# jpe17/TwoTowerMLRetrieval

Hardware: AMD Instinct MI355X
Metric: queries/sec top-k over 10M x 256-d docs (higher is better)
Workload: dtype f32 results (bit-identical to the fp32 FMA chain); f16-MFMA screen + fp32 rescoring

## Files before the change

### twotowermlretrieval_amd/csrc/score_topk.hip

```cpp
#include "tt_common.h"

#include <limits.h>
#include <math.h>

namespace {

constexpr int TILE_DOCS = 32;
constexpr int SLAB_BYTES = 32 * 128;
constexpr int NSTAGE = 4;
#ifndef TT_K4_NT_NSTAGE
#define TT_K4_NT_NSTAGE 4
#endif
constexpr int NSTAGE_NT = TT_K4_NT_NSTAGE;
constexpr int WPB = 4;
constexpr int DMA_PER_SLAB = 4;
constexpr int PACE_R = 16;
constexpr int PACE_POLLS = 400;
constexpr int DRAW_POLLS = 1 << 16;
constexpr int DRAW_GAVE_UP = 0x7fffffff;

typedef __attribute__((address_space(3))) void lds_void;
typedef const __attribute__((address_space(1))) void gbl_void;

struct Cand;
// ... 701 lines not shown
        for (int u = 0; u < MERGE_SEG / MERGE_THREADS; ++u) {
            const int m = base + tid + u * MERGE_THREADS;
            ci[u] = m < end ? ix_at(m) : -1;
        }
#pragma unroll
        for (int u = 0; u < MERGE_SEG / MERGE_THREADS; ++u) {
            if (ci[u] >= 0) {
                const int slot = atomicAdd(&pool_n, 1);
                pool_v[slot] = v_at(base + tid + u * MERGE_THREADS);
                pool_i[slot] = ci[u];
            }
        }
        __syncthreads();
    }
    const int kept = reduce_pool();
    if (tid < k) {
        out_val[(size_t)b * k + tid] = tid < kept ? pool_v[tid] : -INFINITY;
        out_idx[(size_t)b * k + tid] = tid < kept ? pool_i[tid] : -1;
    }
}

__device__ __forceinline__ unsigned order_key(float f)
{
    const unsigned b = __float_as_uint(f);
    return (b & 0x80000000u) ? ~b : (b | 0x80000000u);
}

__device__ __forceinline__ float order_key_to_float(unsigned key)
{
    return __uint_as_float((key & 0x80000000u) ? (key & 0x7fffffffu) : ~key);
}

__global__ __launch_bounds__(256) void kth_largest_kernel(const float *__restrict__ vals, int M, int k,
                                                          float *__restrict__ out, const int *run_if,
                                                          float *__restrict__ top_out)
{
    if (run_if && run_if[blockIdx.x >> 5] == 0)
        return;
    __shared__ int hist[256];
    __shared__ int sel[2];
    __shared__ int wpos;
    const int row = blockIdx.x, tid = threadIdx.x, lane = tid & 63;
    const float *v = vals + (size_t)row * M;
    if (M < k) {
        if (tid == 0 && out)
            out[row] = -INFINITY;
        if (top_out)
            for (int i = tid; i < k; i += 256)
                top_out[(size_t)row * k + i] = i < M ? v[i] : -INFINITY;
        return;
    }
    unsigned prefix = 0u, mask = 0u;
    int k_rem = k;
    constexpr int KTH_REG = 16;
    const bool in_regs = M <= 256 * KTH_REG;
    unsigned keys[KTH_REG];
    if (in_regs) {
#pragma unroll
        for (int i = 0; i < KTH_REG; ++i) {
            const int m = tid + 256 * i;
            keys[i] = m < M ? order_key(v[m]) : 0u;
        }
    }
#pragma unroll 1
    for (int pass = 0; pass < 4; ++pass) {
        const int shift = 24 - 8 * pass;
        hist[tid] = 0;
        __syncthreads();
        if (in_regs) {
#pragma unroll
            for (int i = 0; i < KTH_REG; ++i)
                if (tid + 256 * i < M && (keys[i] & mask) == prefix)
                    atomicAdd(&hist[(keys[i] >> shift) & 255u], 1);
        } else {
            for (int m = tid; m < M; m += 256) {
                const unsigned key = order_key(v[m]);
                if ((key & mask) == prefix)
                    atomicAdd(&hist[(key >> shift) & 255u], 1);
            }
        }
        __syncthreads();
        if (tid < 64) {
            int c[4], s = 0;
#pragma unroll
            for (int i = 0; i < 4; ++i) {
                c[i] = hist[255 - (lane * 4 + i)];
                s += c[i];
            }
            int incl = s;
#pragma unroll
            for (int off = 1; off < 64; off <<= 1) {
                const int y = __shfl_up(incl, off);
                if (lane >= off)
                    incl += y;
            }
            int above = incl - s;
#pragma unroll
            for (int i = 0; i < 4; ++i) {
                if (above < k_rem && above + c[i] >= k_rem) {
                    sel[0] = 255 - (lane * 4 + i);
                    sel[1] = above;
                }
                above += c[i];
            }
        }
        __syncthreads();
        prefix |= (unsigned)sel[0] << shift;
        mask |= 0xffu << shift;
        k_rem -= sel[1];
        __syncthreads();
    }
    const float kth = order_key_to_float(prefix);
    if (tid == 0 && out)
        out[row] = kth;
    if (top_out) {
        if (tid == 0)
            wpos = 0;
        __syncthreads();
        float *dst = top_out + (size_t)row * k;
        if (in_regs) {
#pragma unroll
            for (int i = 0; i < KTH_REG; ++i)
                if (tid + 256 * i < M && keys[i] > prefix)
                    dst[atomicAdd(&wpos, 1)] = order_key_to_float(keys[i]);
        } else {
            for (int m = tid; m < M; m += 256)
// ... 636 lines not shown
```

### twotowermlretrieval_amd/csrc/screen.hip

```cpp
#include "tt_common.h"
#include <cmath>

#include <hip/hip_fp16.h>
#include <limits.h>
#include <math.h>

int tt_score_topk_f32_pred(const float *Q, int B, int d, const float *D, int64_t N, int k, int64_t idx_offset,
                           float *out_val, int64_t *out_idx, void *workspace, size_t workspace_bytes,
                           const int *run_if, hipStream_t st);

int tt_kth_largest(const float *vals, int B, int M, int k, float *out, hipStream_t st);
int tt_k_largest_list(const float *vals, int B, int M, int k, float *list, hipStream_t st);

namespace {

typedef _Float16 h8 __attribute__((ext_vector_type(8)));
typedef _Float16 h4 __attribute__((ext_vector_type(4)));
typedef __attribute__((address_space(3))) void lds_void;
typedef const __attribute__((address_space(1))) void gbl_void;

#ifndef TT_SCREEN_STAGGER
#define TT_SCREEN_STAGGER 1
#endif
constexpr int SW = 8;
constexpr int STILE_BYTES = 32 * 512;
constexpr int SRING = 8;
constexpr int STPB = 2;
constexpr int SCAP = 128;
constexpr int SURV_MAX = 1024;
constexpr int POOL_MAX = 8192;
constexpr int FIN_MAX_CHUNKS = 2048;

struct SCand {
    float v;
    int x;
};

__device__ __forceinline__ float screen_eps(float qnorm, float dmax)
{
    return 1.10e-3f * qnorm * dmax + 1e-6f * (qnorm + dmax);
}

__device__ __forceinline__ SCand scand_load_l2(const SCand *p)
{
    unsigned long long u = __hip_atomic_load((const unsigned long long *)p, __ATOMIC_RELAXED, __HIP_MEMORY_SCOPE_AGENT);
    SCand c;
    c.v = __uint_as_float((unsigned)u);
    c.x = (int)(u >> 32);
    return c;
}

struct ScreenParams {
    const float *Q;
    const _Float16 *D16;
    int B, N, k;
    int n_chunks, tiles_per_chunk, n_tiles;
    int static_tiles, tail_g, tail_blocks;
    int *tail_ctr;
    float dmax;
    SCand *cand;
    int *pcnt;
    int *flag;
    float *max_val;
    const float *thr0;
    int thr0_stride;
    const h8 *qimg;
    const float *qnorm;
    const float *dbg_thr;
};

__device__ __forceinline__ void scand_store_async(const SCand *base, unsigned byte_off, float v, int x)
{
    const unsigned long long bits = ((unsigned long long)(unsigned)x << 32) | (unsigned long long)__float_as_uint(v);
    asm volatile("global_store_dwordx2 %0, %1, %2\n\ts_nop 1" ::"v"(byte_off), "v"(bits), "s"(base) : "memory");
}

__device__ __forceinline__ void f32_store_async(float *dst, float v)
{
    asm volatile("global_store_dword %0, %1, off\n\ts_nop 0" ::"v"(dst), "v"(v) : "memory");
}

constexpr int SQUART = SCAP / 4;
constexpr int SQ_TRIGGER = SQUART - 10;
constexpr int SQ_KEEP_MAX = 4 * SQ_TRIGGER - 4;

__device__ __forceinline__ void screen_compact(SCand *base, const int (&n)[4], int k, float slack, int lane, int &n_new,
                                               float &thr_new, bool &have, bool &overflow)
{
    float v[2];
    int x[2], rank[2];
    bool live[2];
#pragma unroll
    for (int i = 0; i < 2; ++i) {
        v[i] = -INFINITY;
        x[i] = INT_MAX;
        rank[i] = 0;
        live[i] = (lane & 31) < ((lane >> 5) ? n[2 * i + 1] : n[2 * i]);
        if (live[i]) {
            const SCand c = scand_load_l2(base + 64 * i + lane);
            v[i] = c.v;
            x[i] = c.x;
        }
    }
#pragma unroll
    for (int i2 = 0; i2 < 2; ++i2) {
#pragma unroll
        for (int sub = 0; sub < 2; ++sub) {
            const int lim = n[2 * i2 + sub];
            for (int l2 = 0; l2 < lim; ++l2) {
                const float sv = __builtin_bit_cast(float, __builtin_amdgcn_readlane(__builtin_bit_cast(int, v[i2]), 32 * sub + l2));
                const int sx = __builtin_amdgcn_readlane(x[i2], 32 * sub + l2);
#pragma unroll
                for (int i = 0; i < 2; ++i)
                    rank[i] += (sv > v[i] || (sv == v[i] && sx < x[i])) ? 1 : 0;
            }
        }
// ... 118 lines not shown
                            : INFINITY;
        float c_init = -t_init;
        if (MAXONLY)
            c_init = (p.dbg_thr && live) ? -p.dbg_thr[qrow] : 0.0f;
        negthr[c] = f32x4{c_init, c_init, c_init, c_init};
    }

    SCand *const cwave = p.cand + ((size_t)blockIdx.x * QB + w * QW) * SCAP;

    auto compact_where = [&](int c, unsigned qmask) {
        asm volatile("s_waitcnt vmcnt(0)" ::: "memory");
        while (qmask) {
            const int q = __ffs((int)qmask) - 1;
            qmask &= qmask - 1;
            const int nq[4] = {__builtin_amdgcn_readlane(cnt[c], q), __builtin_amdgcn_readlane(cnt[c], q + 16),
                               __builtin_amdgcn_readlane(cnt[c], q + 32), __builtin_amdgcn_readlane(cnt[c], q + 48)};
            const float slack = __builtin_bit_cast(float, __builtin_amdgcn_readlane(__builtin_bit_cast(int, eps2[c]), q));
            int n_new;
            float tn;
            bool have, ovf;
            screen_compact(cwave + (size_t)(16 * c + q) * SCAP, nq, k, slack, lane, n_new, tn, have, ovf);
            if (ovf && lane == 0)
                atomicOr(p.flag + ((qbase + 16 * c) >> 5), 1);
            if (n == q) {
                cnt[c] = (n_new - g + 3) >> 2;
                if (have)
                    negthr[c] = f32x4{-tn, -tn, -tn, -tn};
            }
        }
    };

    const char *D = (const char *)p.D16;
    const char *rowp[2];
    auto set_rows = [&](int tile) {
#pragma unroll
        for (int i = 0; i < 2; ++i) {
            const int row = 2 * (2 * w + i) + (lane >> 5);
            const int doc = min(tile * 32 + row, p.N - 1);
            const int chunk16 = (lane & 31) ^ (row & 15);
            rowp[i] = D + (size_t)doc * 512 + chunk16 * 16;
        }
    };
    auto dma_issue = [&](int tile, int stage) {
        set_rows(min(tile, t1 - 1));
        char *dst = ring + stage * STILE_BYTES + (2 * w) * 1024;
        __builtin_amdgcn_global_load_lds((gbl_void *)rowp[0], (lds_void *)dst, 16, 0, DMA_AUX);
        __builtin_amdgcn_global_load_lds((gbl_void *)rowp[1], (lds_void *)(dst + 1024), 16, 0, DMA_AUX);
    };
    auto dma_piece = [&](int i, int stage) {
        char *dst = ring + stage * STILE_BYTES + (2 * w + i) * 1024;
        __builtin_amdgcn_global_load_lds((gbl_void *)rowp[i], (lds_void *)dst, 16, 0, DMA_AUX);
    };

    for (;;) {
    if (t0 < t1) {
#pragma unroll
        for (int gi = 0; gi < SRING - STPB; ++gi)
            dma_issue(t0 + gi, gi);
        int stage = 0;
        const int rd_base = n * 512;
        f32x4 acc[2][NSET];
        const bool late = TT_SCREEN_STAGGER && w >= 4;
        bool pending = false;
        int ptile = 0;
        auto epilogue = [&](int tile) {
                const int tile_base = tile * 32;
            const bool partial = tile_base + 32 > p.N;
            if (!MAXONLY) {
                if (partial) {
#pragma unroll
                    for (int u = 0; u < 2; ++u)
#pragma unroll
                        for (int r = 0; r < 4; ++r)
                            if (tile_base + 16 * u + 4 * g + r >= p.N) {
#pragma unroll
                                for (int c = 0; c < NSET; ++c)
                                    acc[u][c][r] = -INFINITY;
                            }
                }
                int mall = INT_MIN;
#pragma unroll
                for (int u = 0; u < 2; ++u)
#pragma unroll
                    for (int c = 0; c < NSET; ++c)
#pragma unroll
                        for (int r = 0; r < 4; ++r)
                            mall = max(mall, __float_as_int(acc[u][c][r]));
                if (__ballot(mall >= 0) != 0ull) {
#pragma unroll
                    for (int c = 0; c < NSET; ++c) {
                        int mu[2];
#pragma unroll
                        for (int u = 0; u < 2; ++u)
                            mu[u] = max(max(__float_as_int(acc[u][c][0]), __float_as_int(acc[u][c][1])),
                                        max(__float_as_int(acc[u][c][2]), __float_as_int(acc[u][c][3])));
                        if (__ballot(max(mu[0], mu[1]) >= 0) == 0ull)
                            continue;
                        const unsigned mine = (unsigned)(((16 * c + n) * SCAP + SQUART * g) * sizeof(SCand));
                        const float thr_c = -negthr[c][0];
#pragma unroll
                        for (int u = 0; u < 2; ++u) {
                            if (__ballot(mu[u] >= 0) == 0ull)
                                continue;
#pragma unroll
                            for (int r = 0; r < 4; ++r) {
                                if (__float_as_int(acc[u][c][r]) >= 0) {
                                    scand_store_async(cwave, mine + (unsigned)cnt[c] * (unsigned)sizeof(SCand),
                                                      acc[u][c][r] + thr_c, tile_base + 16 * u + 4 * g + r);
                                    ++cnt[c];
                                }
                            }
                        }
                        unsigned long long full = __ballot(cnt[c] > SQ_TRIGGER);
                        full = (full | (full >> 32));
                        full = (full | (full >> 16)) & 0xffffull;
                        if (full)
                            compact_where(c, (unsigned)full);
                    }
                }
            } else {
#pragma unroll
                for (int c = 0; c < NSET; ++c) {
                    float m = -INFINITY;
                    if (!partial) {
                        int mi = INT_MIN;
#pragma unroll
                        for (int u = 0; u < 2; ++u)
#pragma unroll
                            for (int r = 0; r < 4; ++r)
                                mi = max(mi, __float_as_int(acc[u][c][r]));
                        m = __int_as_float(mi);
                    } else {
#pragma unroll
                        for (int u = 0; u < 2; ++u)
#pragma unroll
                            for (int r = 0; r < 4; ++r)
                                m = fmaxf(m, tile_base + 16 * u + 4 * g + r < p.N ? acc[u][c][r] : -INFINITY);
                    }
                    m = fmaxf(m, __shfl_xor(m, 16));
                    m = fmaxf(m, __shfl_xor(m, 32));
                    const int qrow = qbase + 16 * c + n;
                    if (g == 0 && qrow < p.B)
                        f32_store_async(p.max_val + (size_t)qrow * p.n_tiles + tile, m);
                }
            }
                };
        for (int tile = t0; tile < t1; ++tile) {
            if ((tile - t0) % STPB == 0) {
                asm volatile("s_waitcnt vmcnt(%0)" ::"n"(2 * (SRING - 2 * STPB)) : "memory");
                __builtin_amdgcn_s_barrier();
            }
            const int fill_stage = (stage + SRING - STPB) % SRING;
            set_rows(min(tile + SRING - STPB, t1 - 1));
            if (!wave_live) {
                dma_piece(0, fill_stage);
                dma_piece(1, fill_stage);
            }
            if (wave_live) {
                if (late && pending)
                    epilogue(ptile);
                const char *buf = ring + stage * STILE_BYTES + rd_base;
                h8 a0[3], a1[3];
                auto a_read = [&](int s) {
                    const int off = ((4 * s + g) ^ n) << 4;
                    a0[s % 3] = *(const h8 *)(buf + off);
                    a1[s % 3] = *(const h8 *)(buf + 16 * 512 + off);
                };
                a_read(0);
                a_read(1);
#pragma unroll
                for (int s = 0; s < 8; ++s) {
                    if (s + 2 < 8)
                        a_read(s + 2);
                    if (s == 2)
                        dma_piece(0, fill_stage);
                    if (s == 6)
                        dma_piece(1, fill_stage);
                    __builtin_amdgcn_sched_barrier(0);
#pragma unroll
                    for (int c = 0; c < NSET; ++c) {
                        const f32x4 c0 = s == 0 ? negthr[c] : acc[0][c];
                        const f32x4 c1 = s == 0 ? negthr[c] : acc[1][c];
                        acc[0][c] = __builtin_amdgcn_mfma_f32_16x16x32_f16(a0[s % 3], qreg[c][s], c0, 0, 0, 0);
                        acc[1][c] = __builtin_amdgcn_mfma_f32_16x16x32_f16(a1[s % 3], qreg[c][s], c1, 0, 0, 0);
                    }
                    __builtin_amdgcn_sched_barrier(0);
                }
                if (late) {
                    pending = true;
                    ptile = tile;
                } else {
                    epilogue(tile);
                }
            }
            stage = (stage + 1) % SRING;
        }
// ... 222 lines not shown
                    const int qrow = qbase + 16 * c + n;
                    if (g == 0 && qrow < p.B)
                        f32_store_async(p.max_val + (size_t)qrow * p.n_tiles + tile, m);
                }
            }
        }
    }
    asm volatile("s_waitcnt vmcnt(0)" ::: "memory");
    if (MAXONLY)
        return;
#pragma unroll
    for (int c = 0; c < NQS; ++c) {
        int tot = cnt[c] + __shfl_xor(cnt[c], 16);
        tot += __shfl_xor(tot, 32);
        const unsigned long long over = __ballot(tot > k) & 0xffffull;
        if (over)
            compact_where(c, (unsigned)over);
        int packed = cnt[c] << (8 * g);
        packed |= __shfl_xor(packed, 16);
        packed |= __shfl_xor(packed, 32);
        const int qrow = qbase + 16 * c + n;
        if (g == 0 && qrow < p.B)
            p.pcnt[(size_t)qrow * p.n_chunks + chunk] = packed;
    }
}

struct FinishParams {
    const float *Q;
    const float *D32;
    int B, N, k, n_chunks;
    float dmax;
    const SCand *cand;
    const int *pcnt;
    int *flag;
    int64_t idx_offset;
    float *out_val;
    int64_t *out_idx;
    int q_per_block;
    int *stats;
};

__device__ __forceinline__ bool before_f(float sa, int ia, float sb, int ib) { return sa > sb || (sa == sb && ia < ib); }

__device__ __forceinline__ unsigned f32_order_key(float f)
{
    const unsigned b = __float_as_uint(f);
    return (b & 0x80000000u) ? ~b : (b | 0x80000000u);
}
__device__ __forceinline__ float f32_from_order_key(unsigned k)
{
    return __uint_as_float((k & 0x80000000u) ? (k & 0x7fffffffu) : ~k);
}

__global__ __launch_bounds__(256) void screen_finish_kernel(FinishParams p)
{
    __shared__ float pool_v[POOL_MAX];
    __shared__ float qs[256];
    __shared__ float sv_v[SURV_MAX];
    __shared__ int sv_x[SURV_MAX];
    __shared__ float red_v[4];
    __shared__ int hist[256];
    extern __shared__ int fin_dyn[];
    int *const ccnt = fin_dyn;
    int *const pre = fin_dyn + p.n_chunks;
    __shared__ int sel[2];
    __shared__ int n_pool, n_surv;
    const int row = blockIdx.x, tid = threadIdx.x;
    if (tid == 0)
        n_pool = n_surv = 0;
    qs[tid] = p.Q[(size_t)row * 256 + tid];
    __syncthreads();
    float ss = qs[tid] * qs[tid];
#pragma unroll
    for (int off = 32; off >= 1; off >>= 1)
        ss += __shfl_xor(ss, off);
    if ((tid & 63) == 0)
        red_v[tid >> 6] = ss;
    __syncthreads();
    const float eps2 = 2.0f * screen_eps(sqrtf(red_v[0] + red_v[1] + red_v[2] + red_v[3]), p.dmax);
    __syncthreads();

    const int qgroup = row / p.q_per_block, qin = row % p.q_per_block;
    bool too_many = false;
    const int per = (p.n_chunks + 255) / 256;
    {
        int sum = 0;
        for (int c = tid * per; c < min(tid * per + per, p.n_chunks); ++c) {
            const int v = p.pcnt[(size_t)row * p.n_chunks + c];
            ccnt[c] = v;
            sum += (v & 0xff) + ((v >> 8) & 0xff) + ((v >> 16) & 0xff) + ((v >> 24) & 0xff);
        }
        int inc = sum;
#pragma unroll
        for (int off = 1; off < 64; off <<= 1) {
            const int v = __shfl_up(inc, off);
            if ((tid & 63) >= off)
                inc += v;
        }
        if ((tid & 63) == 63)
            hist[tid >> 6] = inc;
        __syncthreads();
        int base = 0;
        for (int wv = 0; wv < (tid >> 6); ++wv)
            base += hist[wv];
        if (tid == 255)
            n_pool = base + inc;
        __syncthreads();
        hist[tid] = base + inc - sum;
    }
    __syncthreads();
    {
        int run = hist[tid];
        for (int c = tid * per; c < min(tid * per + per, p.n_chunks); ++c) {
            pre[c] = run;
            const int v = ccnt[c];
            run += (v & 0xff) + ((v >> 8) & 0xff) + ((v >> 16) & 0xff) + ((v >> 24) & 0xff);
        }
        if (tid == 255)
            pre[p.n_chunks] = n_pool;
    }
    __syncthreads();
    const int total = n_pool;
    if (total > POOL_MAX)
        too_many = true;
    auto locate = [&](int m) -> const SCand * {
        int lo = 0, hi = p.n_chunks;
        while (hi - lo > 1) {
            const int mid = (lo + hi) >> 1;
            if (pre[mid] <= m)
                lo = mid;
            else
                hi = mid;
        }
        int o = m - pre[lo], slot = 0;
#pragma unroll
        for (int gq = 0; gq < 4; ++gq) {
            const int ng = (ccnt[lo] >> (8 * gq)) & 0xff;
            if (o >= 0 && o < ng)
                slot = SQUART * gq + o;
            o -= ng;
            if (o < 0)
                o = INT_MIN / 2;
        }
        return p.cand + ((size_t)(qgroup * p.n_chunks + lo) * p.q_per_block + qin) * SCAP + slot;
// ... 13 lines not shown
            hist[tid] = 0;
            __syncthreads();
            for (int m = tid; m < np; m += 256) {
                const unsigned key = f32_order_key(pool_v[m]);
                if ((key & mask) == prefix)
                    atomicAdd(&hist[(key >> shift) & 255u], 1);
            }
            __syncthreads();
            if (tid < 64) {
                const int ln = tid;
                int c[4], sm = 0;
#pragma unroll
                for (int i = 0; i < 4; ++i) {
                    c[i] = hist[255 - (ln * 4 + i)];
                    sm += c[i];
                }
                int incl = sm;
#pragma unroll
                for (int off = 1; off < 64; off <<= 1) {
                    const int y = __shfl_up(incl, off);
                    if (ln >= off)
                        incl += y;
                }
                int above = incl - sm;
#pragma unroll
                for (int i = 0; i < 4; ++i) {
                    if (above < k_rem && above + c[i] >= k_rem) {
                        sel[0] = 255 - (ln * 4 + i);
                        sel[1] = above;
                    }
                    above += c[i];
                }
            }
            __syncthreads();
            prefix |= (unsigned)sel[0] << shift;
            mask |= 0xffu << shift;
            k_rem -= sel[1];
            __syncthreads();
        }
        kth = f32_from_order_key(prefix);
    }
    const float cut = found == p.k ? kth - eps2 : -INFINITY;
    for (int m = tid; m < np; m += 256) {
        if (pool_v[m] >= cut) {
            const int slot = atomicAdd(&n_surv, 1);
            if (slot < SURV_MAX)
                sv_x[slot] = locate(m)->x;
            else
                too_many = true;
        }
    }
    __syncthreads();
    const int ns = min(n_surv, SURV_MAX);
    for (int sidx = tid; sidx < ns; sidx += 256) {
        const float *drow = p.D32 + (size_t)sv_x[sidx] * 256;
        float acc = 0.0f;
#pragma unroll 1
        for (int x0 = 0; x0 < 256; x0 += 64) {
            f32x4 dv[16];
#pragma unroll
            for (int i = 0; i < 16; ++i)
                dv[i] = __builtin_nontemporal_load((const f32x4 *)(drow + x0 + 4 * i));
#pragma unroll
            for (int i = 0; i < 16; ++i) {
                acc = fmaf(qs[x0 + 4 * i], dv[i].x, acc);
                acc = fmaf(qs[x0 + 4 * i + 1], dv[i].y, acc);
                acc = fmaf(qs[x0 + 4 * i + 2], dv[i].z, acc);
                acc = fmaf(qs[x0 + 4 * i + 3], dv[i].w, acc);
            }
        }
        sv_v[sidx] = acc;
    }
    if (tid == 0) {
        p.stats[2 * row] = n_pool;
        p.stats[2 * row + 1] = n_surv;
    }
    if (__syncthreads_or(too_many) && tid == 0)
        atomicOr(p.flag + (row >> 5), 4);
    __syncthreads();
    for (int sidx = tid; sidx < ns; sidx += 256) {
        const float mv = sv_v[sidx];
        const int mx = sv_x[sidx];
        int rank = 0;
        for (int u = 0; u < ns; ++u)
            rank += before_f(sv_v[u], sv_x[u], mv, mx) ? 1 : 0;
        if (rank < p.k) {
            p.out_val[(size_t)row * p.k + rank] = mv;
            p.out_idx[(size_t)row * p.k + rank] = p.idx_offset + mx;
        }
    }
    for (int r = ns + tid; r < p.k; r += 256) {
        p.out_val[(size_t)row * p.k + r] = -INFINITY;
        p.out_idx[(size_t)row * p.k + r] = -1;
    }
}

__global__ __launch_bounds__(256) void build_f16_kernel(const float *__restrict__ D, int64_t N, int d,
                                                        _Float16 *__restrict__ out, unsigned *__restrict__ stats)
{
    __shared__ float red[8];
    const int lane = threadIdx.x & 63, wave = threadIdx.x >> 6;
    float nmax = 0.0f, amax = 0.0f;
    for (int64_t row = (int64_t)blockIdx.x * 4 + wave; row < N; row += (int64_t)gridDim.x * 4) {
        float ss = 0.0f;
        for (int x = lane * 4; x < d; x += 256) {
            const f32x4 v = *(const f32x4 *)(D + row * d + x);
            h4 hv;
#pragma unroll
            for (int e = 0; e < 4; ++e) {
                ss += v[e] * v[e];
                amax = fmaxf(amax, fabsf(v[e]));
                if (!(fabsf(v[e]) <= 3.0e38f))
                    amax = INFINITY;
                hv[e] = (_Float16)v[e];
            }
            *(h4 *)(out + row * d + x) = hv;
        }
#pragma unroll
        for (int off = 32; off >= 1; off >>= 1)
            ss += __shfl_xor(ss, off);
        nmax = fmaxf(nmax, sqrtf(ss));
    }
#pragma unroll
    for (int off = 32; off >= 1; off >>= 1)
// ... 17 lines not shown
    const int lane = threadIdx.x & 63, wave = threadIdx.x >> 6;
    float nmax = 0.0f, amax = 0.0f;
    for (int64_t row = (int64_t)blockIdx.x * 4 + wave; row < N; row += (int64_t)gridDim.x * 4) {
        float ss = 0.0f;
        for (int x = lane * 4; x < d; x += 256) {
            const uint2 raw = *(const uint2 *)(S + row * d + x);
            f32x4 v;
            v[0] = __uint_as_float(raw.x << 16);
            v[1] = __uint_as_float(raw.x & 0xffff0000u);
            v[2] = __uint_as_float(raw.y << 16);
            v[3] = __uint_as_float(raw.y & 0xffff0000u);
            h4 hv;
#pragma unroll
            for (int e = 0; e < 4; ++e) {
                ss += v[e] * v[e];
                amax = fmaxf(amax, fabsf(v[e]));
                if (!(fabsf(v[e]) <= 3.0e38f))
                    amax = INFINITY;
                hv[e] = (_Float16)v[e];
            }
            *(f32x4 *)(out32 + row * d + x) = v;
            if (out16)
                *(h4 *)(out16 + row * d + x) = hv;
        }
#pragma unroll
        for (int off = 32; off >= 1; off >>= 1)
            ss += __shfl_xor(ss, off);
        nmax = fmaxf(nmax, sqrtf(ss));
    }
#pragma unroll
    for (int off = 32; off >= 1; off >>= 1)
        amax = fmaxf(amax, __shfl_xor(amax, off));
    if (lane == 0) {
        red[wave] = nmax;
        red[4 + wave] = amax;
    }
    __syncthreads();
    if (threadIdx.x == 0 && stats) {
        atomicMax(stats, __float_as_uint(fmaxf(fmaxf(red[0], red[1]), fmaxf(red[2], red[3]))));
        atomicMax(stats + 1, __float_as_uint(fmaxf(fmaxf(red[4], red[5]), fmaxf(red[6], red[7]))));
    }
}

struct SPlan {
    bool stream;
    int nset;
    int n_qgroups;
    int q_per_block;
    int n_tiles, n_chunks, tiles_per_chunk, n_blocks;
    int static_tiles, tail_g, tail_blocks;
    size_t tailctr_off;
    bool sample;
    int s_tiles, s_chunks, s_tiles_per_chunk, s_blocks;
    int64_t s_docs;
    size_t cand_off, pcnt_off, smax_val_off, sthr_val_off, qimg_off, qnorm_off, stats_off, ws_bytes, lds;
    int rows_pad;
};

constexpr int64_t SAMPLE_MIN_N = 65536;
constexpr int STREAM_MAX_B = 64;

int screen_cus()
{
    int dev = 0, cus = 0;
    if (hipGetDevice(&dev) != hipSuccess ||
        hipDeviceGetAttribute(&cus, hipDeviceAttributeMultiprocessorCount, dev) != hipSuccess || cus <= 0) {
        (void)hipGetLastError();
        cus = 256;
    }
    return cus;
}

SPlan make_splan(int B, int64_t N, int k)
{
    SPlan pl;
    pl.stream = B <= STREAM_MAX_B;
    if (B <= SW * 32) {
        pl.nset = B <= SW * 16 ? 1 : 2;
    } else {
        const int groups = (B + SW * 64 - 1) / (SW * 64);
        pl.nset = (B + groups - 1) / groups <= SW * 48 ? 3 : 4;
    }
    pl.q_per_block = pl.stream ? (B <= 32 ? 32 : 64) : SW * 16 * pl.nset;
    pl.n_qgroups = (B + pl.q_per_block - 1) / pl.q_per_block;
    pl.n_tiles = (int)((N + 31) / 32);
    int want, max_chunks;
    if (pl.stream) {
        want = (screen_cus() * 2 * TW + pl.n_qgroups - 1) / pl.n_qgroups;
        max_chunks = N >= SAMPLE_MIN_N ? FIN_MAX_CHUNKS : POOL_MAX / (k + 16);
    } else {
        want = (screen_cus() + pl.n_qgroups - 1) / pl.n_qgroups;
        max_chunks = POOL_MAX / (k + 16);
        max_chunks = max_chunks > 255 ? 255 : max_chunks;
    }
    want = want > max_chunks ? max_chunks : want;
    want = want > pl.n_tiles ? pl.n_tiles : want;
    want = want < 1 ? 1 : want;
    pl.tiles_per_chunk = (pl.n_tiles + want - 1) / want;
    pl.n_chunks = (pl.n_tiles + pl.tiles_per_chunk - 1) / pl.tiles_per_chunk;
    pl.static_tiles = pl.n_tiles;
    pl.tail_g = 1;
    pl.tail_blocks = 0;
    {
        const int tail_div = TT_AB_SWITCH(TT_SCREEN_TAIL_DIV, 8);
        const int share = tail_div > 0 ? pl.tiles_per_chunk / tail_div : 0;
        if (!pl.stream && share >= 16) {
            const int own = pl.tiles_per_chunk - share;
            int g = share / 4;
            g = g < 8 ? 8 : (g > 32 ? 32 : g);
            pl.tiles_per_chunk = own;
            pl.static_tiles = own * pl.n_chunks < pl.n_tiles ? own * pl.n_chunks : pl.n_tiles;
            pl.tail_g = g;
            pl.tail_blocks = (pl.n_tiles - pl.static_tiles + g - 1) / g;
        }
    }
    const int n_tasks = pl.n_qgroups * pl.n_chunks;
    pl.n_blocks = pl.stream ? (n_tasks + TW - 1) / TW : n_tasks;
    const size_t rows = (size_t)pl.n_qgroups * pl.q_per_block;
    size_t off = 0;
    pl.cand_off = off;
    off = tt_align_up(off + (size_t)n_tasks * pl.q_per_block * SCAP * sizeof(SCand), 256);
    pl.pcnt_off = off;
    off = tt_align_up(off + rows * pl.n_chunks * sizeof(int), 256);
    pl.sample = N >= SAMPLE_MIN_N;
    int64_t s_docs = N / 64;
    const int per_k = k <= 16 ? 4096 : 2048;
    const int64_t s_min = (int64_t)k * per_k < N / 4 ? (int64_t)k * per_k : N / 4;
    s_docs = s_docs < s_min ? s_min : s_docs;
    s_docs = s_docs < 32 ? 32 : s_docs;
    pl.s_docs = (s_docs + 31) / 32 * 32;
    pl.s_tiles = (int)(pl.s_docs / 32);
    int s_want = pl.stream ? (screen_cus() * 2 * TW + pl.n_qgroups - 1) / pl.n_qgroups
                           : (screen_cus() + pl.n_qgroups - 1) / pl.n_qgroups;
    s_want = s_want > pl.s_tiles ? pl.s_tiles : s_want;
    s_want = s_want < 1 ? 1 : s_want;
    pl.s_tiles_per_chunk = (pl.s_tiles + s_want - 1) / s_want;
    pl.s_chunks = pl.sample ? (pl.s_tiles + pl.s_tiles_per_chunk - 1) / pl.s_tiles_per_chunk : 0;
    pl.s_blocks = pl.stream ? (pl.n_qgroups * pl.s_chunks + TW - 1) / TW : pl.n_qgroups * pl.s_chunks;
    pl.smax_val_off = off;
    off = tt_align_up(off + rows * (size_t)(pl.sample ? pl.s_tiles : 1) * sizeof(float), 256);
    pl.sthr_val_off = off;
    off = tt_align_up(off + rows * sizeof(float), 256);
    pl.rows_pad = (int)rows;
    pl.qimg_off = off;
    off = tt_align_up(off + rows * 256 * sizeof(_Float16), 256);
    pl.qnorm_off = off;
    off = tt_align_up(off + rows * sizeof(float), 256);
    pl.tailctr_off = off;
    off = tt_align_up(off + (size_t)pl.n_qgroups * sizeof(int), 256);
    pl.stats_off = off;
    off = tt_align_up(off + rows * 2 * sizeof(int), 256);
    pl.ws_bytes = off;
    pl.lds = pl.stream ? (size_t)TW * TSTAGE * TSLAB_BYTES : (size_t)SRING * STILE_BYTES;
    return pl;
}

}

TT_EXPORT int tt_index_build_f16(const float *D, int64_t N, int d, void *D16, float *stats, tt_stream_t stream)
{
    if (N < 0 || d <= 0 || (d & 3))
        return tt_fail(TT_ERR_BAD_SHAPE, "tt_index_build_f16: N=%lld d=%d", (long long)N, d);
    if (!stats || (N > 0 && (!D || !D16)))
        return tt_fail(TT_ERR_BAD_SHAPE, "tt_index_build_f16: null pointer");
    hipStream_t st = (hipStream_t)stream;
    TT_RC_CHECK(tt_zero_async(stats, 2 * sizeof(float), st));
    if (N == 0)
        return TT_OK;
    const int64_t want_blocks = (N + 3) / 4;
    hipLaunchKernelGGL(build_f16_kernel, dim3((unsigned)(want_blocks > 8192 ? 8192 : want_blocks)), dim3(256), 0, st, D,
                       N, d, (_Float16 *)D16, (unsigned *)stats);
    TT_LAUNCH_CHECK();
    return TT_OK;
}

TT_EXPORT int tt_index_build_from_bf16(const void *D_bf16, int64_t N, int d, float *D32, void *D16, float *stats,
                                       int reset_stats, tt_stream_t stream)
{
    if (N < 0 || d <= 0 || (d & 3))
        return tt_fail(TT_ERR_BAD_SHAPE, "tt_index_build_from_bf16: N=%lld d=%d", (long long)N, d);
    if (N > 0 && (!D_bf16 || !D32))
        return tt_fail(TT_ERR_BAD_SHAPE, "tt_index_build_from_bf16: null pointer");
    hipStream_t st = (hipStream_t)stream;
    if (stats && reset_stats)
        TT_RC_CHECK(tt_zero_async(stats, 2 * sizeof(float), st));
    if (N == 0)
        return TT_OK;
    const int64_t want_blocks = (N + 3) / 4;
    hipLaunchKernelGGL(build_from_bf16_kernel, dim3((unsigned)(want_blocks > 8192 ? 8192 : want_blocks)), dim3(256), 0,
                       st, (const unsigned short *)D_bf16, N, d, D32, (_Float16 *)D16, (unsigned *)stats);
    TT_LAUNCH_CHECK();
    return TT_OK;
}
// ... 14 lines not shown
}

namespace {
__global__ void seed_fill_kernel(float *seed, int n)
{
    const int i = blockIdx.x * 256 + threadIdx.x;
    if (i < n)
        seed[i] = -3.0e38f;
}

int screened_impl(const char *who, int phase, const float *Q, int B, int d, const float *D32, const void *D16, int64_t N, int k,
                  int k_seed, float dmax_norm, int64_t idx_offset, float *out_val, int64_t *out_idx, int32_t *fallback_flag,
                  float *seed, void *workspace, size_t workspace_bytes, void *const *prof_events, hipStream_t st)
{
    if (B <= 0 || N <= 0 || k <= 0)
        return tt_fail(TT_ERR_BAD_SHAPE, "%s: B=%d N=%lld k=%d", who, B, (long long)N, k);
    if (d != 256)
        return tt_fail(TT_ERR_UNSUPPORTED, "%s: d=%d (supported: 256)", who, d);
    if (k > 64)
        return tt_fail(TT_ERR_UNSUPPORTED, "%s: k=%d > 64", who, k);
    if (N >= (int64_t)INT_MAX - 64)
        return tt_fail(TT_ERR_UNSUPPORTED, "%s: N too large; shard the corpus", who);
    if (!(dmax_norm >= 0.0f) || !(dmax_norm < 60000.0f))
        return tt_fail(TT_ERR_UNSUPPORTED, "%s: corpus norm %g outside the fp16 range", who, dmax_norm);
    const bool seed_only = phase == 1 || phase == 3;
    if (!Q || !D16 || !fallback_flag || (!seed_only && (!D32 || !out_val || !out_idx)) || (phase != 0 && !seed))
        return tt_fail(TT_ERR_BAD_SHAPE, "%s: null pointer", who);
    if (seed_only && (k_seed < 1 || k_seed > k))
        return tt_fail(TT_ERR_BAD_SHAPE, "%s: k_seed=%d outside [1, k=%d]", who, k_seed, k);
    const SPlan pl = make_splan(B, N, k);
    const size_t need = pl.ws_bytes + tt_score_topk_workspace_bytes(B, N, d, k);
    if (!workspace || workspace_bytes < need || ((uintptr_t)workspace & 255))
        return tt_fail(TT_ERR_WORKSPACE, "%s: workspace %zu < %zu bytes", who, workspace_bytes, need);
    char *ws = (char *)workspace;

    ScreenParams sp;
    sp.Q = Q;
    sp.D16 = (const _Float16 *)D16;
    sp.B = B;
    sp.N = (int)N;
    sp.k = k;
    sp.n_chunks = pl.n_chunks;
    sp.tiles_per_chunk = pl.tiles_per_chunk;
    sp.n_tiles = pl.n_tiles;
    sp.static_tiles = pl.static_tiles;
    sp.tail_g = pl.tail_g;
    sp.tail_blocks = pl.tail_blocks;
    sp.tail_ctr = (int *)(ws + pl.tailctr_off);
    sp.dmax = dmax_norm;
    sp.cand = (SCand *)(ws + pl.cand_off);
    sp.pcnt = (int *)(ws + pl.pcnt_off);
    sp.flag = fallback_flag;
    sp.max_val = nullptr;
    sp.thr0 = nullptr;
    sp.thr0_stride = k;
    sp.qimg = (const h8 *)(ws + pl.qimg_off);
    sp.qnorm = (const float *)(ws + pl.qnorm_off);
    sp.dbg_thr = nullptr;
    if (phase != 2) {
        hipLaunchKernelGGL(q_image_kernel, dim3(pl.rows_pad / 32), dim3(128), 0, st, Q, B, (h8 *)(ws + pl.qimg_off),
                           (float *)(ws + pl.qnorm_off), fallback_flag, (B + 31) / 32, (int *)(ws + pl.tailctr_off),
                           pl.n_qgroups);
        TT_LAUNCH_CHECK();
    }
    auto launch = [&](const ScreenParams &a, int blocks, bool maxonly) -> int {
        if (pl.stream && pl.q_per_block == 64) {
            if (maxonly)
                hipLaunchKernelGGL((screen_stream_kernel<true, 4>), dim3(blocks), dim3(TW * 64), pl.lds, st, a);
            else
                hipLaunchKernelGGL((screen_stream_kernel<false, 4>), dim3(blocks), dim3(TW * 64), pl.lds, st, a);
        } else if (pl.stream) {
            if (maxonly)
                hipLaunchKernelGGL(screen_stream_kernel<true>, dim3(blocks), dim3(TW * 64), pl.lds, st, a);
            else
                hipLaunchKernelGGL(screen_stream_kernel<false>, dim3(blocks), dim3(TW * 64), pl.lds, st, a);
        } else if (pl.nset == 4) {
            if (maxonly)
                hipLaunchKernelGGL((screen_kernel<true, 4>), dim3(blocks), dim3(SW * 64), pl.lds, st, a);
            else
                hipLaunchKernelGGL((screen_kernel<false, 4>), dim3(blocks), dim3(SW * 64), pl.lds, st, a);
        } else if (pl.nset == 3) {
            if (maxonly)
                hipLaunchKernelGGL((screen_kernel<true, 3>), dim3(blocks), dim3(SW * 64), pl.lds, st, a);
            else
                hipLaunchKernelGGL((screen_kernel<false, 3>), dim3(blocks), dim3(SW * 64), pl.lds, st, a);
        } else if (pl.nset == 2) {
            if (maxonly)
                hipLaunchKernelGGL((screen_kernel<true, 2>), dim3(blocks), dim3(SW * 64), pl.lds, st, a);
            else
                hipLaunchKernelGGL((screen_kernel<false, 2>), dim3(blocks), dim3(SW * 64), pl.lds, st, a);
        } else {
            if (maxonly)
                hipLaunchKernelGGL((screen_kernel<true, 1>), dim3(blocks), dim3(SW * 64), pl.lds, st, a);
            else
                hipLaunchKernelGGL((screen_kernel<false, 1>), dim3(blocks), dim3(SW * 64), pl.lds, st, a);
        }
        TT_LAUNCH_CHECK();
        return TT_OK;
    };
    if (pl.stream && pl.q_per_block == 64) {
        TT_HIP_CHECK(hipFuncSetAttribute((const void *)screen_stream_kernel<false, 4>, hipFuncAttributeMaxDynamicSharedMemorySize, (int)pl.lds));
        TT_HIP_CHECK(hipFuncSetAttribute((const void *)screen_stream_kernel<true, 4>, hipFuncAttributeMaxDynamicSharedMemorySize, (int)pl.lds));
    } else if (pl.stream) {
        TT_HIP_CHECK(hipFuncSetAttribute((const void *)screen_stream_kernel<false>, hipFuncAttributeMaxDynamicSharedMemorySize, (int)pl.lds));
        TT_HIP_CHECK(hipFuncSetAttribute((const void *)screen_stream_kernel<true>, hipFuncAttributeMaxDynamicSharedMemorySize, (int)pl.lds));
    } else {
        const void *fns[8] = {(const void *)screen_kernel<false, 4>, (const void *)screen_kernel<true, 4>,
                              (const void *)screen_kernel<false, 2>, (const void *)screen_kernel<true, 2>,
                              (const void *)screen_kernel<false, 1>, (const void *)screen_kernel<true, 1>,
                              (const void *)screen_kernel<false, 3>, (const void *)screen_kernel<true, 3>};
        const int f0 = pl.nset == 4 ? 0 : (pl.nset == 2 ? 2 : (pl.nset == 3 ? 6 : 4));
        TT_HIP_CHECK(hipFuncSetAttribute(fns[f0], hipFuncAttributeMaxDynamicSharedMemorySize, (int)pl.lds));
        TT_HIP_CHECK(hipFuncSetAttribute(fns[f0 + 1], hipFuncAttributeMaxDynamicSharedMemorySize, (int)pl.lds));
    }
    if (phase == 2) {
        sp.thr0 = seed;
        sp.thr0_stride = 1;
    } else if (!pl.sample && seed_only) {
        const int n = phase == 3 ? B * k_seed : B;
        hipLaunchKernelGGL(seed_fill_kernel, dim3((n + 255) / 256), dim3(256), 0, st, seed, n);
        TT_LAUNCH_CHECK();
    } else if (pl.sample) {
        ScreenParams ss = sp;
        ss.N = (int)pl.s_docs;
        ss.n_tiles = pl.s_tiles;
        ss.n_chunks = pl.s_chunks;
        ss.tiles_per_chunk = pl.s_tiles_per_chunk;
        ss.static_tiles = pl.s_tiles;
        ss.tail_blocks = 0;
        ss.max_val = (float *)(ws + pl.smax_val_off);
        int rc = launch(ss, pl.s_blocks, true);
        if (rc != TT_OK)
            return rc;
        if (phase == 3)
            rc = tt_k_largest_list(ss.max_val, B, pl.s_tiles, k_seed, seed, st);
        else
            rc = tt_kth_largest(ss.max_val, B, pl.s_tiles, phase == 1 ? k_seed : k, phase == 1 ? seed : (float *)(ws + pl.sthr_val_off), st);
        if (rc != TT_OK)
            return rc;
        sp.thr0 = (const float *)(ws + pl.sthr_val_off);
        sp.thr0_stride = 1;
    }
    if (seed_only)
        return TT_OK;
    if (prof_events)
        TT_HIP_CHECK(hipEventRecord((hipEvent_t)prof_events[0], st));
    {
        const int rc = launch(sp, pl.n_blocks, false);
        if (rc != TT_OK)
            return rc;
    }
    if (prof_events)
        TT_HIP_CHECK(hipEventRecord((hipEvent_t)prof_events[1], st));

    FinishParams fp;
    fp.Q = Q;
    fp.D32 = D32;
    fp.B = B;
    fp.N = (int)N;
    fp.k = k;
    fp.n_chunks = pl.n_chunks;
    fp.q_per_block = pl.q_per_block;
    fp.dmax = dmax_norm;
    fp.cand = sp.cand;
    fp.pcnt = sp.pcnt;
    fp.flag = fallback_flag;
    fp.idx_offset = idx_offset;
    fp.out_val = out_val;
    fp.out_idx = out_idx;
    fp.stats = (int *)(ws + pl.stats_off);
    hipLaunchKernelGGL(screen_finish_kernel, dim3(B), dim3(256), (size_t)(2 * pl.n_chunks + 1) * sizeof(int), st, fp);
    TT_LAUNCH_CHECK();
    return tt_score_topk_f32_pred(Q, B, d, D32, N, k, idx_offset, out_val, out_idx, ws + pl.ws_bytes,
                                  workspace_bytes - pl.ws_bytes, fallback_flag, st);
}
}

TT_EXPORT int tt_score_topk_screened_f32(const float *Q, int B, int d, const float *D32, const void *D16, int64_t N,
                                         int k, float dmax_norm, int64_t idx_offset, float *out_val, int64_t *out_idx,
                                         int32_t *fallback_flag, void *workspace, size_t workspace_bytes,
                                         void *const *prof_events, tt_stream_t stream)
{
    return screened_impl("tt_score_topk_screened_f32", 0, Q, B, d, D32, D16, N, k, k, dmax_norm, idx_offset, out_val, out_idx,
                         fallback_flag, nullptr, workspace, workspace_bytes, prof_events, (hipStream_t)stream);
}

TT_EXPORT int tt_score_topk_screened_seed_f32(const float *Q, int B, int d, const void *D16, int64_t N, int k, int k_seed,
                                              float dmax_norm, int32_t *fallback_flag, float *seed, void *workspace,
                                              size_t workspace_bytes, tt_stream_t stream)
{
// ... 40 lines not shown
    pl.n_chunks = (pl.n_tiles + pl.tiles_per_chunk - 1) / pl.tiles_per_chunk;
    const int n_tasks = pl.n_qgroups * pl.n_chunks;
    pl.n_blocks = form == 0 ? (n_tasks + TW - 1) / TW : n_tasks;
    size_t off = 0;
    pl.qimg_off = off;
    off = tt_align_up(off + (size_t)pl.rows_pad * 256 * sizeof(_Float16), 256);
    pl.qnorm_off = off;
    off = tt_align_up(off + (size_t)pl.rows_pad * sizeof(float), 256);
    pl.flag_off = off;
    off = tt_align_up(off + (size_t)(pl.rows_pad / 32 + 1) * sizeof(int), 256);
    pl.total = off;
    return true;
}
}

TT_EXPORT size_t tt_debug_screen_s16_workspace_bytes(int B, int64_t N, int form)
{
    DbgPlan pl;
    if (B <= 0 || N <= 0 || !make_dbg_plan(B, N, form, pl))
        return 0;
    return pl.total;
}

TT_EXPORT int tt_debug_screen_s16(const float *Q, int B, const void *D16, int64_t N, float dmax_norm, const float *thr,
                                  int form, float *out_t, void *workspace, size_t workspace_bytes, tt_stream_t stream)
{
    hipStream_t st = (hipStream_t)stream;
    DbgPlan pl;
    if (B <= 0 || N <= 0 || N >= (int64_t)INT_MAX - 64 || !make_dbg_plan(B, N, form, pl))
        return tt_fail(TT_ERR_BAD_SHAPE, "tt_debug_screen_s16: B=%d N=%lld form=%d", B, (long long)N, form);
    if (!Q || !D16 || !out_t)
        return tt_fail(TT_ERR_BAD_SHAPE, "tt_debug_screen_s16: null pointer");
    if (!workspace || workspace_bytes < pl.total || ((uintptr_t)workspace & 255))
        return tt_fail(TT_ERR_WORKSPACE, "tt_debug_screen_s16: workspace %zu < %zu bytes", workspace_bytes, pl.total);
    char *ws = (char *)workspace;
    ScreenParams sp;
    sp.Q = Q;
    sp.D16 = (const _Float16 *)D16;
    sp.B = B;
    sp.N = (int)N;
    sp.k = 1;
    sp.n_chunks = pl.n_chunks;
    sp.tiles_per_chunk = pl.tiles_per_chunk;
    sp.n_tiles = pl.n_tiles;
    sp.static_tiles = pl.n_tiles;
    sp.tail_g = 1;
    sp.tail_blocks = 0;
    sp.tail_ctr = nullptr;
    sp.dmax = dmax_norm;
    sp.cand = nullptr;
    sp.pcnt = nullptr;
    sp.flag = (int *)(ws + pl.flag_off);
    sp.max_val = out_t;
    sp.thr0 = nullptr;
    sp.thr0_stride = 1;
    sp.qimg = (const h8 *)(ws + pl.qimg_off);
    sp.qnorm = (const float *)(ws + pl.qnorm_off);
    sp.dbg_thr = thr;
    hipLaunchKernelGGL(q_image_kernel, dim3(pl.rows_pad / 32), dim3(128), 0, st, Q, B, (h8 *)(ws + pl.qimg_off),
                       (float *)(ws + pl.qnorm_off), sp.flag, pl.rows_pad / 32, (int *)nullptr, 0);
    TT_LAUNCH_CHECK();
    if (form == 0) {
        const size_t lds = (size_t)TW * TSTAGE * TSLAB_BYTES;
        TT_HIP_CHECK(hipFuncSetAttribute((const void *)screen_stream_kernel<true>, hipFuncAttributeMaxDynamicSharedMemorySize, (int)lds));
        hipLaunchKernelGGL(screen_stream_kernel<true>, dim3(pl.n_blocks), dim3(TW * 64), lds, st, sp);
    } else {
        const size_t lds = (size_t)SRING * STILE_BYTES;
        const void *fn = form == 4 ? (const void *)screen_kernel<true, 4>
                                   : (form == 2 ? (const void *)screen_kernel<true, 2> : (const void *)screen_kernel<true, 1>);
        TT_HIP_CHECK(hipFuncSetAttribute(fn, hipFuncAttributeMaxDynamicSharedMemorySize, (int)lds));
        if (form == 4)
            hipLaunchKernelGGL((screen_kernel<true, 4>), dim3(pl.n_blocks), dim3(SW * 64), lds, st, sp);
        else if (form == 2)
            hipLaunchKernelGGL((screen_kernel<true, 2>), dim3(pl.n_blocks), dim3(SW * 64), lds, st, sp);
        else
            hipLaunchKernelGGL((screen_kernel<true, 1>), dim3(pl.n_blocks), dim3(SW * 64), lds, st, sp);
    }
    TT_LAUNCH_CHECK();
    return TT_OK;
}
```

Before: 257,700.

## Group sample tile maxima, stage rescoring rows in LDS, and batch histogram atomics

The sampling pass now reduces per-tile maxima over groups of four tiles before storing them, so the kth-largest and list kernels scan a quarter as many values. The kth kernel keeps more keys in registers and merges runs of identical bins into a single atomic. The finish kernel's fp32 rescoring stages survivor rows cooperatively into LDS with coalesced loads instead of having each thread stream its own row, and it hoists the pcnt read ahead of the first barrier. Grouping maxima changes the seed threshold statistics, since a max over four tiles gives a looser kth estimate, and this may let more candidates through.

```diff
diff --git a/twotowermlretrieval_amd/csrc/score_topk.hip b/twotowermlretrieval_amd/csrc/score_topk.hip
--- a/twotowermlretrieval_amd/csrc/score_topk.hip
+++ b/twotowermlretrieval_amd/csrc/score_topk.hip
@@ -777,7 +777,7 @@
     }
     unsigned prefix = 0u, mask = 0u;
     int k_rem = k;
-    constexpr int KTH_REG = 16;
+    constexpr int KTH_REG = 24;
     const bool in_regs = M <= 256 * KTH_REG;
     unsigned keys[KTH_REG];
     if (in_regs) {
@@ -793,10 +793,20 @@
         hist[tid] = 0;
         __syncthreads();
         if (in_regs) {
+            int run_bin = -1, run = 0;
 #pragma unroll
             for (int i = 0; i < KTH_REG; ++i)
-                if (tid + 256 * i < M && (keys[i] & mask) == prefix)
-                    atomicAdd(&hist[(keys[i] >> shift) & 255u], 1);
+                if (tid + 256 * i < M && (keys[i] & mask) == prefix) {
+                    const int bin = (int)((keys[i] >> shift) & 255u);
+                    if (run_bin < 0)
+                        run_bin = bin;
+                    if (bin == run_bin)
+                        ++run;
+                    else
+                        atomicAdd(&hist[bin], 1);
+                }
+            if (run)
+                atomicAdd(&hist[run_bin], run);
         } else {
             for (int m = tid; m < M; m += 256) {
                 const unsigned key = order_key(v[m]);
diff --git a/twotowermlretrieval_amd/csrc/screen.hip b/twotowermlretrieval_amd/csrc/screen.hip
--- a/twotowermlretrieval_amd/csrc/screen.hip
+++ b/twotowermlretrieval_amd/csrc/screen.hip
@@ -62,6 +62,8 @@
     int *pcnt;
     int *flag;
     float *max_val;
+    int max_group;
+    int max_stride;
     const float *thr0;
     int thr0_stride;
     const h8 *qimg;
@@ -286,6 +288,11 @@
         __builtin_amdgcn_global_load_lds((gbl_void *)rowp[i], (lds_void *)dst, 16, 0, DMA_AUX);
     };
 
+    float gmax[NSET];
+#pragma unroll
+    for (int c = 0; c < NSET; ++c)
+        gmax[c] = -INFINITY;
+
     for (;;) {
     if (t0 < t1) {
 #pragma unroll
@@ -353,6 +360,7 @@
                     }
                 }
             } else {
+                const bool flush = p.max_group == 1 || (tile + 1) % p.max_group == 0 || tile + 1 == t1;
 #pragma unroll
                 for (int c = 0; c < NSET; ++c) {
                     float m = -INFINITY;
@@ -370,12 +378,19 @@
 #pragma unroll
                             for (int r = 0; r < 4; ++r)
                                 m = fmaxf(m, tile_base + 16 * u + 4 * g + r < p.N ? acc[u][c][r] : -INFINITY);
+                    }
+                    if (p.max_group > 1) {
+                        gmax[c] = fmaxf(gmax[c], m);
+                        if (!flush)
+                            continue;
+                        m = gmax[c];
+                        gmax[c] = -INFINITY;
                     }
                     m = fmaxf(m, __shfl_xor(m, 16));
                     m = fmaxf(m, __shfl_xor(m, 32));
                     const int qrow = qbase + 16 * c + n;
                     if (g == 0 && qrow < p.B)
-                        f32_store_async(p.max_val + (size_t)qrow * p.n_tiles + tile, m);
+                        f32_store_async(p.max_val + (size_t)qrow * p.max_stride + tile / p.max_group, m);
                 }
             }
                 };
@@ -704,11 +719,14 @@
     return __uint_as_float((k & 0x80000000u) ? (k & 0x7fffffffu) : ~k);
 }
 
+constexpr int RS_STRIDE = 260;
+constexpr int RS_ROWS = (POOL_MAX - SURV_MAX) / RS_STRIDE;
+static_assert(RS_ROWS >= 1 && RS_ROWS * 64 <= 7 * 256, "a staging round is at most 7 row loads per thread");
+
 __global__ __launch_bounds__(256) void screen_finish_kernel(FinishParams p)
 {
-    __shared__ float pool_v[POOL_MAX];
+    __shared__ __attribute__((aligned(16))) float pool_v[POOL_MAX];
     __shared__ float qs[256];
-    __shared__ float sv_v[SURV_MAX];
     __shared__ int sv_x[SURV_MAX];
     __shared__ float red_v[4];
     __shared__ int hist[256];
@@ -721,6 +739,13 @@
     if (tid == 0)
         n_pool = n_surv = 0;
     qs[tid] = p.Q[(size_t)row * 256 + tid];
+    const int per = (p.n_chunks + 255) / 256;
+    int sum = 0;
+    for (int c = tid * per; c < min(tid * per + per, p.n_chunks); ++c) {
+        const int v = p.pcnt[(size_t)row * p.n_chunks + c];
+        ccnt[c] = v;
+        sum += (v & 0xff) + ((v >> 8) & 0xff) + ((v >> 16) & 0xff) + ((v >> 24) & 0xff);
+    }
     __syncthreads();
     float ss = qs[tid] * qs[tid];
 #pragma unroll
@@ -734,14 +759,7 @@
 
     const int qgroup = row / p.q_per_block, qin = row % p.q_per_block;
     bool too_many = false;
-    const int per = (p.n_chunks + 255) / 256;
     {
-        int sum = 0;
-        for (int c = tid * per; c < min(tid * per + per, p.n_chunks); ++c) {
-            const int v = p.pcnt[(size_t)row * p.n_chunks + c];
-            ccnt[c] = v;
-            sum += (v & 0xff) + ((v >> 8) & 0xff) + ((v >> 16) & 0xff) + ((v >> 24) & 0xff);
-        }
         int inc = sum;
 #pragma unroll
         for (int off = 1; off < 64; off <<= 1) {
@@ -861,24 +879,38 @@
     }
     __syncthreads();
     const int ns = min(n_surv, SURV_MAX);
-    for (int sidx = tid; sidx < ns; sidx += 256) {
-        const float *drow = p.D32 + (size_t)sv_x[sidx] * 256;
-        float acc = 0.0f;
-#pragma unroll 1
-        for (int x0 = 0; x0 < 256; x0 += 64) {
-            f32x4 dv[16];
-#pragma unroll
-            for (int i = 0; i < 16; ++i)
-                dv[i] = __builtin_nontemporal_load((const f32x4 *)(drow + x0 + 4 * i));
-#pragma unroll
-            for (int i = 0; i < 16; ++i) {
-                acc = fmaf(qs[x0 + 4 * i], dv[i].x, acc);
-                acc = fmaf(qs[x0 + 4 * i + 1], dv[i].y, acc);
-                acc = fmaf(qs[x0 + 4 * i + 2], dv[i].z, acc);
-                acc = fmaf(qs[x0 + 4 * i + 3], dv[i].w, acc);
+    float *const stage = pool_v;
+    float *const sv_v = pool_v + RS_ROWS * RS_STRIDE;
+    for (int b0 = 0; b0 < ns; b0 += RS_ROWS) {
+        const int nb = min(RS_ROWS, ns - b0);
+        f32x4 dv[7];
+#pragma unroll
+        for (int i = 0; i < 7; ++i) {
+            const int e = tid + 256 * i;
+            if (e < nb * 64)
+                dv[i] = __builtin_nontemporal_load((const f32x4 *)(p.D32 + (size_t)sv_x[b0 + (e >> 6)] * 256) + (e & 63));
+        }
+#pragma unroll
+        for (int i = 0; i < 7; ++i) {
+            const int e = tid + 256 * i;
+            if (e < nb * 64)
+                *(f32x4 *)(stage + (e >> 6) * RS_STRIDE + 4 * (e & 63)) = dv[i];
+        }
+        __syncthreads();
+        if (tid < nb) {
+            const float *srow = stage + tid * RS_STRIDE;
+            float acc = 0.0f;
+#pragma unroll 8
+            for (int x = 0; x < 256; x += 4) {
+                const f32x4 d4 = *(const f32x4 *)(srow + x);
+                acc = fmaf(qs[x], d4.x, acc);
+                acc = fmaf(qs[x + 1], d4.y, acc);
+                acc = fmaf(qs[x + 2], d4.z, acc);
+                acc = fmaf(qs[x + 3], d4.w, acc);
             }
-        }
-        sv_v[sidx] = acc;
+            sv_v[b0 + tid] = acc;
+        }
+        __syncthreads();
     }
     if (tid == 0) {
         p.stats[2 * row] = n_pool;
@@ -1002,12 +1034,14 @@
     size_t tailctr_off;
     bool sample;
     int s_tiles, s_chunks, s_tiles_per_chunk, s_blocks;
+    int s_group, s_groups;
     int64_t s_docs;
     size_t cand_off, pcnt_off, smax_val_off, sthr_val_off, qimg_off, qnorm_off, stats_off, ws_bytes, lds;
     int rows_pad;
 };
 
 constexpr int64_t SAMPLE_MIN_N = 65536;
+constexpr int SGROUP = 4;
 constexpr int STREAM_MAX_B = 64;
 
 int screen_cus()
@@ -1084,11 +1118,14 @@
                            : (screen_cus() + pl.n_qgroups - 1) / pl.n_qgroups;
     s_want = s_want > pl.s_tiles ? pl.s_tiles : s_want;
     s_want = s_want < 1 ? 1 : s_want;
+    pl.s_group = pl.stream ? 1 : SGROUP;
     pl.s_tiles_per_chunk = (pl.s_tiles + s_want - 1) / s_want;
+    pl.s_tiles_per_chunk = (pl.s_tiles_per_chunk + pl.s_group - 1) / pl.s_group * pl.s_group;
+    pl.s_groups = (pl.s_tiles + pl.s_group - 1) / pl.s_group;
     pl.s_chunks = pl.sample ? (pl.s_tiles + pl.s_tiles_per_chunk - 1) / pl.s_tiles_per_chunk : 0;
     pl.s_blocks = pl.stream ? (pl.n_qgroups * pl.s_chunks + TW - 1) / TW : pl.n_qgroups * pl.s_chunks;
     pl.smax_val_off = off;
-    off = tt_align_up(off + rows * (size_t)(pl.sample ? pl.s_tiles : 1) * sizeof(float), 256);
+    off = tt_align_up(off + rows * (size_t)(pl.sample ? pl.s_groups : 1) * sizeof(float), 256);
     pl.sthr_val_off = off;
     off = tt_align_up(off + rows * sizeof(float), 256);
     pl.rows_pad = (int)rows;
@@ -1209,6 +1246,8 @@
     sp.pcnt = (int *)(ws + pl.pcnt_off);
     sp.flag = fallback_flag;
     sp.max_val = nullptr;
+    sp.max_group = 1;
+    sp.max_stride = 0;
     sp.thr0 = nullptr;
     sp.thr0_stride = k;
     sp.qimg = (const h8 *)(ws + pl.qimg_off);
@@ -1286,13 +1325,15 @@
         ss.static_tiles = pl.s_tiles;
         ss.tail_blocks = 0;
         ss.max_val = (float *)(ws + pl.smax_val_off);
+        ss.max_group = pl.s_group;
+        ss.max_stride = pl.s_groups;
         int rc = launch(ss, pl.s_blocks, true);
         if (rc != TT_OK)
             return rc;
         if (phase == 3)
-            rc = tt_k_largest_list(ss.max_val, B, pl.s_tiles, k_seed, seed, st);
+            rc = tt_k_largest_list(ss.max_val, B, pl.s_groups, k_seed, seed, st);
         else
-            rc = tt_kth_largest(ss.max_val, B, pl.s_tiles, phase == 1 ? k_seed : k, phase == 1 ? seed : (float *)(ws + pl.sthr_val_off), st);
+            rc = tt_kth_largest(ss.max_val, B, pl.s_groups, phase == 1 ? k_seed : k, phase == 1 ? seed : (float *)(ws + pl.sthr_val_off), st);
         if (rc != TT_OK)
             return rc;
         sp.thr0 = (const float *)(ws + pl.sthr_val_off);
@@ -1439,6 +1480,8 @@
     sp.pcnt = nullptr;
     sp.flag = (int *)(ws + pl.flag_off);
     sp.max_val = out_t;
+    sp.max_group = 1;
+    sp.max_stride = pl.n_tiles;
     sp.thr0 = nullptr;
     sp.thr0_stride = 1;
     sp.qimg = (const h8 *)(ws + pl.qimg_off);
```

Result: faster. 261,200, median of 6 (+1.4%).
